# igorshmukler/kokoro-ruslan

Measured on AMD Instinct MI355X. Metric: mel-frames/sec (full train step), higher is better.
Workload: dtype bf16; 1 GPU; kokoro acoustic-model train step, 8x512 mel frames x 64 phonemes per GPU (BASELINE configs[1]), 49.4M params, fwd+loss+bwd+clip+AdamW+EMA every step; global_batch=8, frames=512, phonemes=64, parallelism=dp1, grad_allreduce=none (1 GPU), grad_accumulation=1, hipgraph=True

## Files before the change

### include/kokoro_hip.h

```cpp
#ifndef KOKORO_HIP_H
#define KOKORO_HIP_H
#include <stdint.h>
#ifdef __cplusplus
extern "C" {
#endif

#define KK_ABI_VERSION 2
#define KK_MATH_F32 0
#define KK_MATH_BF16 1
#define KK_EINVAL (-22)
#define KK_ENOTSUP (-95)
#define KK_SEG_ALIGN 1024

int kk_abi_version(void);
const char *kk_last_error(void);
const char *kk_last_kernel(void);

int kk_gemm(int ta, int tb, int64_t M, int64_t N, int64_t K, float alpha, const float *A, int64_t lda,
            const float *B, int64_t ldb, float beta, float *C, int64_t ldc, const float *bias,
            const float *residual, int64_t ldr, int64_t res_mod, int split_k, int math, int dtypes,
            void *stream);
typedef struct {
    const void *dy; int64_t lddy;
    const void *x;  int64_t ldx;
// ... 297 lines not shown
    double ema_decay;
    double max_weight_norm;
    int64_t ema_update_every;
    int64_t legacy_schedule;
    double legacy_cos, eta_min;
} KkOptCfg;
#define KK_OS_SKIPPED 0
#define KK_OS_EXPL_EMA 1
#define KK_OS_EXPL_EMA_STEPS 2
#define KK_OS_EXPL_STREAK 3
#define KK_OS_LAST_GRAD_NORM 4
#define KK_OS_LAST_CLIP_COEF 5
#define KK_OS_LAST_SKIP 6
#define KK_OS_LAST_BASE_LR 7
#define KK_OS_LAST_CLIP_NORM 8
#define KK_OS_EXPL_EMA_VALID 9
#define KK_OS_ATTEMPT 10
#define KK_OS_BAD_SEG 11
#define KK_OS_BAD_COUNT 12
#define KK_OS_BAD_ATTEMPT 13
#define KK_OS_MICRO_BAD 14
#define KK_OS_MICRO_BAD_TOTAL 15
#define KK_OS_SIZE 16
int64_t kk_seg_sumsq_ws_bytes(int64_t nblocks);
int64_t kk_seg_sumsq_rec_offset(void);
int kk_seg_sumsq_rec_capacity(void);
int kk_seg_sumsq(const float *buf, const int32_t *block_seg, int64_t nblocks, double *sumsq, int nseg, void *ws,
                 const int32_t *seg_skip, int extra_records, void *stream);
int kk_opt_prepare(const double *grad_sumsq, const float *seg_preclip, const float *seg_lr_mult,
                   const float *seg_wd, int nseg, const int64_t *max_dur, const KkOptCfg *cfg,
                   double *opt_state, float *seg_gscale, float *seg_decay, float *seg_stepsize,
                   float *step_consts ,
                   double *clear_a, double *clear_b , void *stream);
int kk_adamw_ema(float *p, const float *g, float *m, float *v, float *ema, const int32_t *block_seg,
                 int64_t nblocks, const float *seg_gscale, const float *seg_decay, const float *seg_stepsize,
                 const int32_t *seg_flags, const float *step_consts, float beta1, float beta2,
                 float ema_decay, int64_t *p_sumsq, int nseg, void *p_bf16, int zeroed, void *stream);
int kk_weight_norm_project(float *p, const int32_t *block_seg, int64_t nblocks, const int64_t *p_sumsq ,
                           const int32_t *seg_flags, const float *step_consts, double max_norm, void *p_bf16,
                           void *stream);
int kk_cast_f32_bf16(const float *src, void *dst, int64_t n, void *stream);

int kk_chain_begin(void *stream);
int kk_chain_launch(int kind, uint32_t *sync, uint64_t *trace, int flags, void *stream);
int kk_chain_abort(void *stream);

int kk_comm_load(const char *rccl_path );
int kk_comm_unique_id(void *id128);
int kk_comm_init(int rank, int world, const void *nccl_unique_id);
int kk_comm_world(void);
int kk_comm_destroy(void);
int kk_comm_reduce_bucket(void *ptr, int64_t count, int dtype, void *comm_stream);
int kk_comm_reduce_ranges(void *base, const int64_t *begin, const int64_t *end, int n, int dtype, void *comm_stream);
int kk_comm_loss_sync(double *acc, int n_acc, int64_t *max_dur, void *stream);
int kk_comm_reduce_scatter(const void *send, void *recv, int64_t recv_count, int dtype, void *comm_stream);
int kk_comm_all_gather(const void *send, void *recv, int64_t send_count, int dtype, void *comm_stream);
int kk_cast_bf16_f32(const void *x, float *y, int64_t n, float scale, void *stream);
int kk_cast_ranges(const void *src, void *dst, const int64_t *begin, const int64_t *end, int n, int to_bf16, float scale,
                   void *stream);

int kk_timestamp(uint64_t *slot, void *stream);
int kk_copy_many(const void *const *src, void *const *dst, const int64_t *bytes, int n, void *stream);
int kk_zero_many(void *const *dst, const int64_t *bytes, int n, void *stream);
int kk_axpby(float a, const float *x, float b, float *y, int64_t n, void *stream);
int kk_mfma_probe(float *out_f32 , float *out_bf16 , void *stream);

// ... 5 lines not shown
```

### include/kokoro_hip_tuning.h

```cpp
#ifndef KOKORO_HIP_TUNING_H
#define KOKORO_HIP_TUNING_H
#ifdef __cplusplus
extern "C" {
#endif
int kk_gemm_tune(int tm_threshold, int xcd_swizzle);
int kk_gemm_tune16(int enable, int thr128, int thr12864, int split_target);
int kk_gemm_tune_group(int split);
int kk_gemm_tune16x(int on, int force, int dbg);
#ifdef __cplusplus
}
#endif
#endif
```

### kokoro_ruslan_amd/csrc/kk_optim.hip

```cpp
#include "kk_common.h"
#include <math.h>

namespace {

constexpr int BLK = KK_SEG_ALIGN;
constexpr double KK_PSUMSQ_ONE = 1073741824.0;

typedef KkSegRec SegRec;
constexpr int SEG_REC_EXTRA = 4096;
constexpr int SEG_SUMSQ_WGS = 2048;

__global__ __launch_bounds__(256) void seg_sumsq_kernel(const float *__restrict__ buf, const int32_t *__restrict__ block_seg,
                                                        int64_t nblocks, int per_wg, double *__restrict__ sumsq, SegRec *__restrict__ rec,
                                                        const int32_t *__restrict__ skip) {
    __shared__ double red[4];
    __shared__ int32_t segs[256], skips[256];
    const int64_t beg = (int64_t)blockIdx.x * per_wg;
    const int64_t end = beg + per_wg < nblocks ? beg + per_wg : nblocks;
    SegRec lead = {0.0, -1, 0}, trail = {0.0, -1, 0};
    if (beg < end) {
        if (threadIdx.x < end - beg) {
            const int sg = block_seg[beg + threadIdx.x];
            segs[threadIdx.x] = sg;
            skips[threadIdx.x] = skip != nullptr ? skip[sg] : 0;
        }
        __syncthreads();
        int cur = segs[0];
        bool first = true;
        double acc = 0.0;
        bool cur_skip = skips[0] != 0;
        for (int64_t blk = beg; blk < end; ++blk) {
            const int seg = segs[blk - beg];
            if (seg != cur) {
                if (!cur_skip) {
                    const double tot = block_sum_256_d(acc, red);
                    if (first) { lead.v = tot; lead.seg = cur; first = false; }
                    else if (threadIdx.x == 0) sumsq[cur] = tot;
                }
                cur = seg;
                cur_skip = skips[blk - beg] != 0;
                acc = 0.0;
            }
            if (cur_skip) continue;
            const float4 v = ld4(buf + blk * BLK + threadIdx.x * 4);
            acc += (double)(v.x * v.x + v.y * v.y) + (double)(v.z * v.z + v.w * v.w);
        }
        if (!cur_skip) {
            const double tot = block_sum_256_d(acc, red);
            if (first) { lead.v = tot; lead.seg = cur; }
            else { trail.v = tot; trail.seg = cur; }
        }
    }
    if (threadIdx.x == 0) {
        rec[2 * blockIdx.x] = lead;
        rec[2 * blockIdx.x + 1] = trail;
    }
}

__device__ __forceinline__ void seg_merge16(const SegRec *in, int n, SegRec *out, double *sumsq, int t, bool last) {
    SegRec a = {0.0, -1, 0}, b = {0.0, -1, 0};
    int cur = -1;
    double acc = 0.0;
    bool have_first = false;
    for (int i = 16 * t; i < 16 * t + 16 && i < n; ++i) {
        const SegRec r = in[i];
        if (r.seg < 0) continue;
        if (r.seg != cur) {
            if (cur >= 0) {
                if (!have_first && !last) { a.v = acc; a.seg = cur; have_first = true; }
                else sumsq[cur] = acc;
            }
            cur = r.seg;
            acc = 0.0;
        }
        acc += r.v;
    }
    if (cur >= 0) {
        if (last) sumsq[cur] = acc;
        else if (!have_first) { a.v = acc; a.seg = cur; }
        else { b.v = acc; b.seg = cur; }
    }
    if (!last) { out[2 * t] = a; out[2 * t + 1] = b; }
}
__global__ __launch_bounds__(512) void seg_sumsq_finish_kernel(const SegRec *__restrict__ rec, int nrec, double *__restrict__ sumsq) {
    __shared__ SegRec l1[1024], l2[128], l3[16], l4[2];
    const int t = threadIdx.x;
    seg_merge16(rec, nrec, l1, sumsq, t, false);
    __syncthreads();
    if (t < 64) seg_merge16(l1, 1024, l2, sumsq, t, false);
    __syncthreads();
    if (t < 8) seg_merge16(l2, 128, l3, sumsq, t, false);
    __syncthreads();
    if (t == 0) seg_merge16(l3, 16, l4, sumsq, 0, true);
}

__device__ double onecycle_lr(const KkOptCfg &c, int64_t step_num) {
    const double total = (double)c.onecycle_steps;
    const double initial = c.max_lr / c.div_factor, min_lr = initial / c.final_div_factor;
    const double end1 = c.pct_start * total - 1.0, end2 = total - 1.0;
    const double PI = 3.14159265358979323846;
    if ((double)step_num <= end1) {
        if (end1 <= 0) return c.max_lr;
        return (initial - c.max_lr) / 2.0 * (cos(PI * ((double)step_num / end1)) + 1.0) + c.max_lr;
    }
    if (end2 <= end1) return min_lr;
    return (c.max_lr - min_lr) / 2.0 * (cos(PI * (((double)step_num - end1) / (end2 - end1))) + 1.0) + min_lr;
}

__device__ double base_lr_for(const KkOptCfg &c, int64_t k) {
    if (k == 0) return onecycle_lr(c, 0);
    const int64_t j = k - 1;
    if (c.use_warmup && j < c.warmup_steps)
        return c.warmup_start_lr + (c.warmup_target_lr - c.warmup_start_lr) * ((double)j / (double)c.warmup_steps);
    int64_t s = c.use_warmup ? j - c.warmup_steps + 1 : j + 1;
    if (s > c.onecycle_steps) s = c.onecycle_steps;
    return onecycle_lr(c, s);
}

__global__ __launch_bounds__(256) void opt_prepare_kernel(const double *__restrict__ grad_sumsq, const float *__restrict__ seg_preclip,
                                                          const float *__restrict__ seg_lr_mult, const float *__restrict__ seg_wd,
                                                          int nseg, const int64_t *__restrict__ max_dur, KkOptCfg c,
                                                          double *__restrict__ st, float *__restrict__ seg_gscale,
                                                          float *__restrict__ seg_decay, float *__restrict__ seg_stepsize,
                                                          float *__restrict__ step_consts, double *clear_a, double *clear_b) {
    __shared__ double red[4];
    __shared__ double sh[4];
    double part = 0.0, bad = 0.0;
    __shared__ int first_bad;
    if (threadIdx.x == 0) first_bad = 0x7fffffff;
    __syncthreads();
    for (int i = threadIdx.x; i < nseg; i += 256) {
        const double ss = grad_sumsq[i];
        const bool fin = isfinite(ss);
        if (!fin) atomicMin(&first_bad, i);
        double nr = sqrt(ss), sc = 1.0;
        const double pre = (double)seg_preclip[i];
        if (pre > 0.0 && fin && nr > pre) sc = pre / (nr + 1e-12);
        seg_gscale[i] = (float)sc;
        nr *= sc;
        part += nr * nr;
        if (!fin) bad += 1.0;
    }
    const double tot2 = block_sum_256_d(part, red);
    const double nbad = block_sum_256_d(bad, red);
    if (threadIdx.x == 0) {
        const double total = sqrt(tot2);
        double clip = c.max_grad_norm;
        const double md = max_dur ? (double)(*max_dur) : 0.0;
        const double risk = fmax((double)c.mel_length / 1400.0, md / 150.0);
        if (risk > 1.0) {
            clip = fmin(clip, fmax(0.3, 0.8 / pow(risk, 0.35)));
            clip = fmax(0.05, 0.5 / sqrt(risk));
        }
        const double attempt = st[KK_OS_ATTEMPT];
        const double done = attempt - st[KK_OS_SKIPPED];
        double floor_ = c.expl_abs_floor;
        if (c.expl_warmup_steps > 0 && done < (double)c.expl_warmup_steps)
            floor_ = c.expl_warmup_floor - (c.expl_warmup_floor - c.expl_abs_floor) * (done / (double)c.expl_warmup_steps);
        const bool ema_valid = st[KK_OS_EXPL_EMA_VALID] != 0.0;
        const bool ema_ready = st[KK_OS_EXPL_EMA_STEPS] >= (double)c.expl_min_ema_steps;
        const double ema_thr = ema_valid ? st[KK_OS_EXPL_EMA] * c.expl_multiplier : 0.0;
// ... 9 lines not shown
        const double coef = fmin(1.0, clip / (total + 1e-6));
        const double blr = c.legacy_schedule ? c.eta_min + (c.learning_rate - c.eta_min) * c.legacy_cos : base_lr_for(c, k);
        sh[0] = coef; sh[1] = blr; sh[2] = 1.0 - pow(c.beta1, (double)(k + 1)); sh[3] = skip ? 1.0 : 0.0;
        step_consts[0] = skip ? 1.f : (c.ema_update_every > 1 && k % c.ema_update_every != 0) ? 2.f : 0.f;
        step_consts[1] = (float)sqrt(1.0 - pow(c.beta2, (double)(k + 1)));
        step_consts[2] = (float)c.eps;
        step_consts[3] = (float)blr;
        st[KK_OS_ATTEMPT] = attempt + 1.0;
        if (skip) {
            st[KK_OS_SKIPPED] += 1.0;
            st[KK_OS_BAD_SEG] = (double)(first_bad + 1);
            st[KK_OS_BAD_COUNT] = nbad;
            st[KK_OS_BAD_ATTEMPT] = attempt;
        }
        st[KK_OS_LAST_GRAD_NORM] = total;
        st[KK_OS_LAST_CLIP_COEF] = coef;
        st[KK_OS_LAST_SKIP] = skip ? 1.0 : 0.0;
        st[KK_OS_LAST_BASE_LR] = blr;
        st[KK_OS_LAST_CLIP_NORM] = clip;
    }
    __syncthreads();
    const double coef = sh[0], blr = sh[1], bc1 = sh[2];
    for (int i = threadIdx.x; i < nseg; i += 256) {
        const double lr = c.legacy_schedule ? c.eta_min + (c.learning_rate * (double)seg_lr_mult[i] - c.eta_min) * c.legacy_cos
                                              : blr * (double)seg_lr_mult[i];
        seg_gscale[i] = (float)((double)seg_gscale[i] * coef);
        seg_decay[i] = (float)(1.0 - lr * (double)seg_wd[i]);
        seg_stepsize[i] = (float)(lr / bc1);
        if (clear_a) clear_a[i] = 0.0;
        if (clear_b) clear_b[i] = 0.0;
    }
}

__global__ __launch_bounds__(256) void adamw_ema_kernel(float *__restrict__ p, const float *__restrict__ g, float *__restrict__ m,
                                                        float *__restrict__ v, float *__restrict__ ema,
                                                        const int32_t *__restrict__ block_seg, const float *__restrict__ seg_gscale,
                                                        const float *__restrict__ seg_decay, const float *__restrict__ seg_stepsize,
                                                        const int32_t *__restrict__ seg_flags, const float *__restrict__ step_consts,
                                                        float beta1, float beta2, float ema_decay, unsigned long long *__restrict__ p_sumsq,
                                                        __bf16 *__restrict__ p16) {
    __shared__ float red[4];
    const float mode = step_consts[0];
    if (mode == 1.f) return;
    const int64_t blk = blockIdx.x;
    const int seg = block_seg[blk];
    const int flags = seg_flags[seg];
    const int64_t o = blk * BLK + threadIdx.x * 4;
    float4 pv = ld4(p + o);
    if (flags & 1) {
        const float gs = seg_gscale[seg], decay = seg_decay[seg], step = seg_stepsize[seg];
        const float bc2s = step_consts[1], eps = step_consts[2];
        const float4 gv = ld4(g + o);
        float4 mv = ld4(m + o), vv = ld4(v + o);
        float *pp = reinterpret_cast<float *>(&pv), *mp = reinterpret_cast<float *>(&mv), *vp = reinterpret_cast<float *>(&vv);
        const float *gp = reinterpret_cast<const float *>(&gv);
#pragma unroll
        for (int e = 0; e < 4; ++e) {
            const float gr = gp[e] * gs;
            float pe = pp[e] * decay;
            mp[e] = mp[e] + (1.f - beta1) * (gr - mp[e]);
            vp[e] = vp[e] * beta2 + (1.f - beta2) * gr * gr;
            const float denom = sqrtf(vp[e]) / bc2s + eps;
            pe = pe - step * (mp[e] / denom);
            pp[e] = pe;
        }
        st4(p + o, pv);
        st4(m + o, mv);
        st4(v + o, vv);
        if (p16) stv4<__bf16>(p16 + o, pv);
    }
    if ((flags & 2) && ema && mode == 0.f) {
        float4 ev = ld4(ema + o);
        const float w = 1.f - ema_decay;
        ev.x = ev.x * ema_decay + pv.x * w;
        ev.y = ev.y * ema_decay + pv.y * w;
        ev.z = ev.z * ema_decay + pv.z * w;
        ev.w = ev.w * ema_decay + pv.w * w;
        st4(ema + o, ev);
    }
    if ((flags & 4) && p_sumsq) {
        const float s = block_sum_256(pv.x * pv.x + pv.y * pv.y + pv.z * pv.z + pv.w * pv.w, red);
        if (threadIdx.x == 0) {
            const float sc = s < 4194304.f ? s : 4194304.f;
            atomicAdd(&p_sumsq[seg], (unsigned long long)((double)sc * KK_PSUMSQ_ONE + 0.5));
        }
    }
}

constexpr int WNP_BLOCKS = 8;
__global__ __launch_bounds__(256) void weight_norm_project_kernel(float *__restrict__ p, const int32_t *__restrict__ block_seg,
                                                                  const unsigned long long *__restrict__ p_sumsq, const int32_t *__restrict__ seg_flags,
                                                                  const float *__restrict__ step_consts, double max_norm,
                                                                  __bf16 *__restrict__ p16, int64_t nblocks) {
    __shared__ float scale[WNP_BLOCKS];
    if (step_consts[0] == 1.f) return;
    const int64_t b0 = (int64_t)blockIdx.x * WNP_BLOCKS;
    if (threadIdx.x < WNP_BLOCKS) {
        float sc = 0.f;
        const int64_t blk = b0 + threadIdx.x;
        if (blk < nblocks) {
            const int seg = block_seg[blk];
            if (seg_flags[seg] & 4) {
                const double nr = sqrt((double)p_sumsq[seg] * (1.0 / KK_PSUMSQ_ONE));
                if (nr > max_norm) sc = (float)(max_norm / nr);
            }
        }
        scale[threadIdx.x] = sc;
    }
    __syncthreads();
#pragma unroll
    for (int j = 0; j < WNP_BLOCKS; ++j) {
        const float sc = scale[j];
        if (sc == 0.f) continue;
        const int64_t o = (b0 + j) * BLK + threadIdx.x * 4;
        float4 pv = ld4(p + o);
        pv.x *= sc; pv.y *= sc; pv.z *= sc; pv.w *= sc;
        st4(p + o, pv);
        if (p16) stv4<__bf16>(p16 + o, pv);
    }
}

__global__ __launch_bounds__(256) void cast_bf16_kernel(const float *__restrict__ src, __bf16 *__restrict__ dst, int64_t n4) {
    for (int64_t i = (int64_t)blockIdx.x * 256 + threadIdx.x; i < n4; i += (int64_t)gridDim.x * 256) stv4<__bf16>(dst + 4 * i, ld4(src + 4 * i));
}

}

extern "C" int64_t kk_seg_sumsq_ws_bytes(int64_t nblocks) {
    (void)nblocks;
    return (int64_t)sizeof(SegRec) * (2 * SEG_SUMSQ_WGS + SEG_REC_EXTRA);
}
extern "C" int64_t kk_seg_sumsq_rec_offset(void) { return (int64_t)sizeof(SegRec) * 2 * SEG_SUMSQ_WGS; }
extern "C" int kk_seg_sumsq_rec_capacity(void) { return SEG_REC_EXTRA; }

extern "C" int kk_seg_sumsq(const float *buf, const int32_t *block_seg, int64_t nblocks, double *sumsq, int nseg, void *ws,
                            const int32_t *seg_skip, int extra_records, void *stream) {
    KK_REQUIRE(buf && block_seg && sumsq && ws && nblocks > 0 && nseg > 0, "kk_seg_sumsq: bad args (the record workspace is required)");
    KK_REQUIRE(extra_records >= 0 && extra_records <= SEG_REC_EXTRA && (extra_records == 0 || seg_skip != nullptr),
               "kk_seg_sumsq: %d tile records (0..%d, with a skip table)", extra_records, SEG_REC_EXTRA);
    hipStream_t s = (hipStream_t)stream;
    const int wgs = SEG_SUMSQ_WGS;
    const int per = kk_cdiv(nblocks, wgs);
    KK_REQUIRE(per <= 256, "kk_seg_sumsq: arenas beyond %d blocks are not supported", 256 * SEG_SUMSQ_WGS);
    SegRec *rec = static_cast<SegRec *>(ws);
    hipLaunchKernelGGL(seg_sumsq_kernel, dim3(wgs), dim3(256), 0, s, buf, block_seg, nblocks, per, sumsq, rec, seg_skip);
    hipLaunchKernelGGL(seg_sumsq_finish_kernel, dim3(1), dim3(512), 0, s, rec, 2 * SEG_SUMSQ_WGS + extra_records, sumsq);
    KK_LAUNCH_CHECK("kk_seg_sumsq");
    return 0;
}

extern "C" int kk_opt_prepare(const double *grad_sumsq, const float *seg_preclip, const float *seg_lr_mult,
                              const float *seg_wd, int nseg, const int64_t *max_dur, const KkOptCfg *cfg,
                              double *opt_state, float *seg_gscale, float *seg_decay, float *seg_stepsize,
                              float *step_consts, double *clear_a, double *clear_b, void *stream) {
    KK_REQUIRE(grad_sumsq && seg_preclip && seg_lr_mult && seg_wd && cfg && opt_state && nseg > 0, "kk_opt_prepare: bad args");
    hipLaunchKernelGGL(opt_prepare_kernel, dim3(1), dim3(256), 0, (hipStream_t)stream, grad_sumsq, seg_preclip, seg_lr_mult,
                       seg_wd, nseg, max_dur, *cfg, opt_state, seg_gscale, seg_decay, seg_stepsize, step_consts, clear_a, clear_b);
    KK_LAUNCH_CHECK("kk_opt_prepare");
    return 0;
}

extern "C" int kk_adamw_ema(float *p, const float *g, float *m, float *v, float *ema, const int32_t *block_seg,
                            int64_t nblocks, const float *seg_gscale, const float *seg_decay,
                            const float *seg_stepsize, const int32_t *seg_flags, const float *step_consts,
                            float beta1, float beta2, float ema_decay, int64_t *p_sumsq, int nseg, void *p_bf16,
                            int zeroed, void *stream) {
    KK_REQUIRE(p && g && m && v && block_seg && nblocks > 0 && nblocks < (1ll << 31), "kk_adamw_ema: bad args");
    hipStream_t s = (hipStream_t)stream;
    if (p_sumsq && !zeroed) {
        const int e = kk_zero_async(p_sumsq, sizeof(int64_t) * nseg, s);
        if (e != 0) return e;
    }
    hipLaunchKernelGGL(adamw_ema_kernel, dim3((unsigned)nblocks), dim3(256), 0, s, p, g, m, v, ema, block_seg, seg_gscale,
                       seg_decay, seg_stepsize, seg_flags, step_consts, beta1, beta2, ema_decay, reinterpret_cast<unsigned long long *>(p_sumsq),
                       reinterpret_cast<__bf16 *>(p_bf16));
    KK_LAUNCH_CHECK("kk_adamw_ema");
    return 0;
}

extern "C" int kk_weight_norm_project(float *p, const int32_t *block_seg, int64_t nblocks, const int64_t *p_sumsq,
                                      const int32_t *seg_flags, const float *step_consts, double max_norm,
                                      void *p_bf16, void *stream) {
    KK_REQUIRE(p && block_seg && p_sumsq && seg_flags && nblocks > 0, "kk_weight_norm_project: bad args");
    if (!(max_norm > 0.0)) return 0;
    hipLaunchKernelGGL(weight_norm_project_kernel, dim3((unsigned)kk_cdiv(nblocks, WNP_BLOCKS)), dim3(256), 0, (hipStream_t)stream, p,
                       block_seg, reinterpret_cast<const unsigned long long *>(p_sumsq), seg_flags, step_consts, max_norm,
                       reinterpret_cast<__bf16 *>(p_bf16), nblocks);
    KK_LAUNCH_CHECK("kk_weight_norm_project");
    return 0;
}

extern "C" int kk_cast_f32_bf16(const float *src, void *dst, int64_t n, void *stream) {
    KK_REQUIRE(src && dst && n > 0 && n % 4 == 0, "kk_cast_f32_bf16: n must be a positive multiple of 4");
    int blocks = kk_cdiv(n / 4, 256);
    if (blocks > 4096) blocks = 4096;
    hipLaunchKernelGGL(cast_bf16_kernel, dim3(blocks), dim3(256), 0, (hipStream_t)stream, src, reinterpret_cast<__bf16 *>(dst), n / 4);
    KK_LAUNCH_CHECK("kk_cast_f32_bf16");
    return 0;
}
```

### kokoro_ruslan_amd/engine.py

```python
from __future__ import annotations

import contextlib
import math
import os
import threading
from collections import OrderedDict
from typing import Dict, Optional, Sequence, Tuple

import torch

from . import lib as kk
from . import spec
from .spec import VA, ModelDims, StepHyper

CHUNK = 512
_ITEMSIZE = {torch.float32: 4, torch.bfloat16: 2, torch.float64: 8, torch.int64: 8, torch.int32: 4, torch.uint8: 1}


def _b16(t) -> int:
    return 1 if t is not None and t.dtype == torch.bfloat16 else 0


class Arena:

# ... 108 lines not shown
        self.train_dropout = False
        self.overlap = True
        self._side = torch.cuda.Stream(device=self.device)
        self._tmp_ns = ""
        self._kv = torch.cuda.Stream(device=self.device)
        self.dec_head_aside = True
        self.tail_aside = -1
        self.embed_bwd_sorted = True
        self.wgrad0_aside = -1
        self.lr_epoch = 0
        self.fuse_glu_fwd = True
        self.group_wgrads = True
        self.fuse_headnorm = True
        self.fuse_headnorm_bwd = True
        self.attn_bwd_pair = True
        self.attn_two_pass = True
        self.attn_keep_bits = True
        self.attn_keep_gen = True
        self.attn_keep_gen_rate = 1100.0
        self.grad_norm_from_wgrads = True
        self._ss_step = None
        self._ss_ready = None
        self._ss_masks: Dict[frozenset, torch.Tensor] = {}
        self._external_sync = False
        self._seg_of_ptr = {self.arena.G[n].data_ptr(): i for i, n in enumerate(self.arena.names)}
        self.attn_warm = 5
        self._keep_ready = set()
        self.attn_pair_min_seq = 64
        self.attn_proj_bf16 = True
        self.fuse_linear_tail = True
        self._acc_clean = True
        self._acc_depth = 0
        self._self_cleaning_acc = True
        self.fuse_enc_prologue = True
        self.rowdot_partials = True
        self.fuse_memory_fwd = True
        self.zero_skip_overwritten = True
        self._ow_sets: Dict[Tuple, frozenset] = {}
        self._ow_seen: Optional[set] = None
        self._ow_expect: Optional[frozenset] = None
        self._wgrad_queue = {}
        self._defer_wgrads = None
        self._grads_fresh = False
        self._first_micro = False
        self.enc_fused = True
        self.enc_fused_max_batch = 8
        self.zero_late = True
        self.enc_placement = 0
        self._enc_sync = torch.zeros(512, dtype=torch.int32, device=self.device)
        self.enc_trace, self.enc_trace_wg = None, 0
        self.spec_augment_active = True
        self.trace = os.environ.get("KK_TRACE", "0") == "1"
        self._marks: Dict[str, int] = {}
        self._mark_buf = torch.zeros(512, dtype=torch.int64, device=self.device) if self.trace else None
        self.rng = torch.full((1,), int(seed) & 0x7FFFFFFF, dtype=torch.int32, device=self.device)
        for n, b in spec.make_buffers(self.dims).items():
            self.arena.P[n].copy_(b)
        if init:
            self.load_params(spec.init_params(self.dims, seed))
        elif self.arena.ema is not None:
            self.arena.ema.copy_(self.arena.p)
        self.sync_shadow()

    @property
    def self_cleaning_acc(self) -> bool:
        return self._self_cleaning_acc

    @self_cleaning_acc.setter
    def self_cleaning_acc(self, on) -> None:
        if bool(on) != self._self_cleaning_acc:
            self._acc_clean = False
        self._self_cleaning_acc = bool(on)

    @contextlib.contextmanager
    def _acc_guard(self):
        if self._acc_depth == 0:
            if not self._acc_clean:
                if torch.cuda.is_current_stream_capturing():
                    raise RuntimeError("the step's accumulators are not in their zero state inside a graph capture")
                self.loss_acc.zero_()
                self.grad_sumsq.zero_()
                self.p_sumsq.zero_()
            self._acc_clean = False
        self._acc_depth += 1
        try:
            yield
        except BaseException:
            self._acc_depth -= 1
            raise
        self._acc_depth -= 1
        if self._acc_depth == 0:
            self._acc_clean = True

    def load_params(self, params: Dict[str, torch.Tensor], reset_ema: bool = True) -> None:
        for n in self.arena.param_names:
            self.arena.P[n].copy_(params[n].to(self.device, torch.float32).view(self.arena.shapes[n]))
        if reset_ema and self.arena.ema is not None:
            self.arena.ema.copy_(self.arena.p)
        self.sync_shadow()

    @contextlib.contextmanager
    def fp32_math(self):
        saved = (self.math, self.enc_dt, self.dec_dt, self.use_shadow)
        self.math, self.enc_dt, self.dec_dt, self.use_shadow = kk.KK_MATH_F32, torch.float32, torch.float32, False
        try:
            yield self
        finally:
            self.math, self.enc_dt, self.dec_dt, self.use_shadow = saved

    @contextlib.contextmanager
    def ema_weights(self):
        a = self.arena
        if a.ema is None:
            yield self
            return
# ... 1364 lines not shown
            self.zero_grad()
            return
        self._ow_expect = rec

        def build():
            base, spans, pos = a.g.data_ptr(), [], 0
            for ptr, n in sorted(rec):
                b = (ptr - base) // 4
                if b < pos or b % 4 or n % 4:
                    raise RuntimeError("overlapping or misaligned weight-gradient tensors in the overwrite record")
                if b > pos:
                    spans.append(a.g[pos:b])
                pos = b + n
            if pos < a.total:
                spans.append(a.g[pos:a.total])
            return [kk.zero_table(spans[i:i + 160]) for i in range(0, len(spans), 160)]
        for dst, nbytes, n in self._table(("zero", a.g.data_ptr(), rec), build):
            kk.call("kk_zero_many", dst, nbytes, n)

    def optimizer_step(self, mel_length: int, tile_norms=None) -> None:
        a, hp = self.arena, self.hp
        cfg = self._opt_cfg(mel_length)
        self._mark("optimizer start")
        skip, extra = None, 0
        if tile_norms is not None and tile_norms[1] > 0:
            skip = self._ss_masks.get(tile_norms[0])
            if skip is None and not torch.cuda.is_current_stream_capturing():
                m = torch.zeros(a.nseg, dtype=torch.int32)
                m[sorted(tile_norms[0])] = 1
                skip = self._ss_masks[tile_norms[0]] = m.to(self.device)
            extra = tile_norms[1] if skip is not None else 0
        with self._acc_guard():
            sc = 1 if self.self_cleaning_acc else 0
            kk.call("kk_seg_sumsq", a.g, a.block_seg, a.nblocks, self.grad_sumsq, a.nseg, self.sumsq_ws, skip, extra)
            kk.call("kk_opt_prepare", self.grad_sumsq, a.seg_preclip, a.seg_lr_mult, a.seg_wd, a.nseg, self.max_dur, cfg,
                    self.opt_state, self.seg_gscale, self.seg_decay, self.seg_stepsize, self.step_consts,
                    None, self.p_sumsq if sc else None)
            kk.call("kk_adamw_ema", a.p, a.g, a.m, a.v, a.ema, a.block_seg, a.nblocks, self.seg_gscale, self.seg_decay,
                    self.seg_stepsize, a.seg_flags, self.step_consts, hp.adam_betas[0], hp.adam_betas[1], hp.ema_decay,
                    self.p_sumsq, a.nseg, a.p16, sc)
            kk.call("kk_weight_norm_project", a.p, a.block_seg, a.nblocks, self.p_sumsq, a.seg_flags, self.step_consts,
                    float(hp.dec_ffn_max_weight_norm), a.p16)
        self._mark("optimizer done")

    def train_step(self, batch: Dict[str, torch.Tensor], accumulation_divisor: Optional[int] = None,
                   boundary: Optional[bool] = None, grad_sync=None, expanded_len: Optional[int] = None) -> torch.Tensor:
        G = max(1, int(self.hp.gradient_accumulation_steps))
        div = accumulation_divisor if accumulation_divisor is not None else G
        if self.micro_in_cycle == 0:
            self.zero_grad()
        is_boundary = bool(boundary) if boundary is not None else self.micro_in_cycle + 1 >= G
        self._exchange_now = is_boundary
        self._first_micro = self.micro_in_cycle == 0
        self._external_sync = grad_sync is not None
        try:
            out = self.forward_backward(batch, loss_scale=self.dp_loss_scale / div, adaptive=True, expanded_len=expanded_len)
        finally:
            self._first_micro = False
            self._external_sync = False
        self._exchange_now = True
        self.micro_in_cycle += 1
        if is_boundary:
            if grad_sync is not None:
                grad_sync(self.arena.g)
            self.optimizer_step(canonical_mel_length(self.global_mel_length, batch["mel_specs"].shape[1]),
                                self._ss_ready if grad_sync is None else None)
            self._ss_ready = None
            self.micro_in_cycle = 0
        return out["losses"]

# ... 65 lines not shown
            if v.data_ptr() == d.data_ptr():
                continue
            if v.shape == d.shape and v.dtype == d.dtype and v.device == d.device and v.is_contiguous() and d.is_contiguous():
                moved.append((d, v))
            else:
                d.copy_(v, non_blocking=True)
        if moved:
            kk.copy_many(moved)
        fkey = (div, first, self.train_dropout, self.spec_augment_active, self.math, self.dp_comm is not None and is_boundary,
                mel_length if self.loss_sync is not None else 0, self.loss_sync is not None, self.self_cleaning_acc, (self.attn_keep_gen, self.attn_keep_gen_rate),
                self.grad_norm_from_wgrads and grad_sync is None)
        with self._acc_guard():
            fbe = ent["fb"].get(fkey)
            if fbe is None:
                with self.capture_lock:
                    self._external_sync = grad_sync is not None
                    try:
                        g_ = self._capture_fb(static, scale, first, expanded_len)
                    finally:
                        self._external_sync = False
                    fbe = ent["fb"][fkey] = (g_, self._ss_ready)
            self._exchange_now = True
            fbe[0].replay()
            self._ss_ready = fbe[1]
        self.micro_in_cycle += 1
        if grad_sync is not None and is_boundary:
            grad_sync(self.arena.g)
        if is_boundary:
            epoch = 0 if self.hp.use_onecycle_lr else self.lr_epoch
            tn = self._ss_ready if grad_sync is None else None
            self._ss_ready = None
            if tn is not None and tn[0] not in self._ss_masks:
                tn = None
            okey = (mel_length, epoch, self.self_cleaning_acc, tn)
            for k in [k for k in ent["opt"] if k[1] != epoch]:
                torch.cuda.synchronize(self.device)
                del ent["opt"][k]
            with self._acc_guard():
                opt = ent["opt"].get(okey)
                if opt is None:
                    with self.capture_lock:
                        torch.cuda.synchronize()
                        opt = ent["opt"][okey] = torch.cuda.CUDAGraph()
                        with torch.cuda.graph(opt, capture_error_mode="thread_local"):
                            self.optimizer_step(mel_length, tn)
                opt.replay()
            self.micro_in_cycle = 0
        return self.losses

    def encoder_stack_error(self) -> int:
        return int(self._enc_sync[0].item())

    def check_encoder_stack(self) -> None:
        import torch.distributed as dist
        multi = dist.is_available() and dist.is_initialized() and dist.get_world_size() > 1
        if not self.enc_fused and not multi:
            return
        code = self.encoder_stack_error() if self.enc_fused else 0
        if multi:
            word = torch.tensor([code], dtype=torch.int64, device=self.device if dist.get_backend() == "nccl" else "cpu")
            dist.all_reduce(word, op=dist.ReduceOp.MAX)
            code = int(word.item())
        if code:
            self._enc_sync.zero_()
            if self.enc_fused:
                self.enc_fused = False
                self._graphs.clear()
# ... 8 lines not shown
```

### kokoro_ruslan_amd/lib.py

```python
from __future__ import annotations

import ctypes as C
import os
from typing import Any, Dict, List

import torch

HERE = os.path.dirname(os.path.abspath(__file__))
LIB_PATH = os.path.join(HERE, "libkokoro_hip.so")

KK_MATH_F32, KK_MATH_BF16 = 0, 1
KK_SEG_ALIGN = 1024
OS = dict(SKIPPED=0, EXPL_EMA=1, EXPL_EMA_STEPS=2, EXPL_STREAK=3, LAST_GRAD_NORM=4, LAST_CLIP_COEF=5,
          LAST_SKIP=6, LAST_BASE_LR=7, LAST_CLIP_NORM=8, EXPL_EMA_VALID=9, ATTEMPT=10, BAD_SEG=11, BAD_COUNT=12,
          BAD_ATTEMPT=13, MICRO_BAD=14, MICRO_BAD_TOTAL=15, SIZE=16)


class KkLossCfg(C.Structure):
    _fields_ = [("w_dur", C.c_float), ("w_stop", C.c_float), ("w_pitch", C.c_float), ("w_energy", C.c_float),
                ("delta_dur", C.c_float), ("delta_pitch", C.c_float), ("delta_energy", C.c_float),
                ("pos_weight", C.c_float), ("loss_scale", C.c_float), ("adaptive", C.c_int)]


class KkOptCfg(C.Structure):
# ... 177 lines not shown
    "kk_encoder_stack_fwd": [C.POINTER(KkEncStack), _P],
    "kk_dropout_bwd": [_P, _P, _L, _I, _I, _P, _U, _F, _U, _F, _U, _F, _I, _P],
    "kk_specaug": [_P, _I, _I, _I, _P, _U, _I, _I, _I, _I, _I, _P],
    "kk_ids_eq_zero": [_P, _P, _L, _P],
    "kk_shift_right": [_P, _P, _I, _I, _I, _P],
    "kk_decode_prologue": [_P, _P, _P, _P, _P, _P, _P, _P, _P, _P, _I, _I, _I, _I, _P],
    "kk_decode_cache_append": [_P, _P, _P, _P, _P, _I, _I, _I, _P],
    "kk_decode_epilogue": [_P, _P, _P, _P, _P, _I, _I, _I, _P],
    "kk_im2col3_rows_fwd": [_P, _P, _P, _I, _I, _I, _I, _I, _P],
    "kk_groupnorm_relu_rows_fwd": [_P, _P, _P, _P, _P, _P, _P, _I, _I, _I, _I, _P, _U, _F, _P],
    "kk_varpred_row_mask": [_P, _P, _P, _I, _I, _I, _P],
    "kk_decode_epilogue_rows": [_P, _P, _P, _P, _P, _P, _P, _P, _P, _P, _P, _I, _I, _I, _F, _F, _P],
    "kk_voc_conv1d": [_P, _L, _I, _P, _I, _I, _P, _P, _I, _I, _I, _F, _P, _I, _P, _P, _I, _I, _P],
    "kk_voc_convt1d": [_P, _L, _I, _P, _I, _I, _P, _P, _I, _I, _I, _F, _P, _I, _I, _P],
    "kk_voc_convt_taps": [_I, _I, _P],
    "kk_voc_post": [_P, _L, _I, _P, _P, _P, _I, _F, _P, _I, _P],
    "kk_gl_tile_frames": [],
    "kk_gl_init": [_P, _L, _P, _P, _P, _P, _P, _P],
    "kk_gl_iter": [_P, _P, _P, _P, _P, _I, _P, _P, _F, _P],
    "kk_gl_istft": [_P, _P, _I, _P, _P, _P, _P],
    "kk_feat_mel_tile_frames": [],
    "kk_feat_peak": [_P, _P, _I, _L, _P, _P],
    "kk_feat_mel": [_P, _P, _P, _P, _P, _I, _P, _P, _P, _P, _P, _P, _P, _P],
    "kk_feat_pitch": [_P, _P, _P, _P, _P, _I, _P, _P, _P, _P, _P],
    "kk_feat_finish": [_P, _P, _I, _P, _P, _P, _P, _P, _P, _P, _P, _I, _P],
    "kk_losses_fwd": [_P] * 12 + [_I, _I, _I, _I, C.POINTER(KkLossCfg), _P, _P, _P, _P, _P, _I, _P],
    "kk_losses_finalize": [_P, C.POINTER(KkLossCfg), _P, _I, _P, _P, _P, _I, _P],
    "kk_losses_bwd": [_P] * 12 + [_I, _I, _I, _I, C.POINTER(KkLossCfg), _P, _P, _P, _P, _P, _P, _P],
    "kk_chain_begin": [_P],
    "kk_chain_launch": [_I, _P, _P, _I, _P],
    "kk_chain_abort": [_P],
    "kk_seg_sumsq": [_P, _P, _L, _P, _I, _P, _P, _I, _P],
    "kk_opt_prepare": [_P, _P, _P, _P, _I, _P, C.POINTER(KkOptCfg), _P, _P, _P, _P, _P, _P, _P, _P],
    "kk_adamw_ema": [_P, _P, _P, _P, _P, _P, _L, _P, _P, _P, _P, _P, _F, _F, _F, _P, _I, _P, _I, _P],
    "kk_weight_norm_project": [_P, _P, _L, _P, _P, _P, _D, _P, _P],
    "kk_cast_f32_bf16": [_P, _P, _L, _P],
    "kk_comm_load": [C.c_char_p],
    "kk_comm_unique_id": [_P],
    "kk_comm_init": [_I, _I, _P],
    "kk_comm_world": [],
    "kk_comm_destroy": [],
    "kk_comm_reduce_bucket": [_P, _L, _I, _P],
    "kk_comm_reduce_ranges": [_P, _P, _P, _I, _I, _P],
    "kk_comm_loss_sync": [_P, _I, _P, _P],
    "kk_comm_reduce_scatter": [_P, _P, _L, _I, _P],
    "kk_comm_all_gather": [_P, _P, _L, _I, _P],
    "kk_cast_bf16_f32": [_P, _P, _L, _F, _P],
    "kk_cast_ranges": [_P, _P, _P, _P, _I, _I, _F, _P],
    "kk_copy_many": [_P, _P, _P, _I, _P],
    "kk_axpby": [_F, _P, _F, _P, _L, _P],
    "kk_timestamp": [_P, _P],
    "kk_mfma_probe": [_P, _P, _P],
}

_lib = None
_prof = None


def profile_start() -> None:
    global _prof
    _prof = []


def profile_stop():
    global _prof
    rec, _prof = _prof or [], None
# ... 105 lines not shown
```

Measured before the change: 1.167 million mel-frames/s.

## Fuse grad segment norm and optimizer prepare into one last-block kernel

Merges the per-segment gradient sum-of-squares walk, the record merge and opt_prepare into one kernel: the last workgroup, found through an atomic ticket, does the merge and the prepare. This removes one or two launches and their serialization gaps. It also prefetches 8 blocks ahead in the segment walk and rewrites the AdamW kernel as a grid-strided loop with next-block prefetch, with optional non-temporal stores. By default the AdamW grid still equals nblocks and temporal stores are used. The ticket needs zeroing in the workspace tail, and correctness relies on threadfence ordering.

Result: slower. 1.144 million mel-frames/s (-2.0%).

```diff
diff --git a/include/kokoro_hip.h b/include/kokoro_hip.h
--- a/include/kokoro_hip.h
+++ b/include/kokoro_hip.h
@@ -353,6 +353,10 @@
                    double *opt_state, float *seg_gscale, float *seg_decay, float *seg_stepsize,
                    float *step_consts ,
                    double *clear_a, double *clear_b , void *stream);
+int kk_opt_norm_prepare(const float *buf, const int32_t *block_seg, int64_t nblocks, double *grad_sumsq, int nseg, void *ws,
+                        const int32_t *seg_skip, int extra_records, const float *seg_preclip, const float *seg_lr_mult,
+                        const float *seg_wd, const int64_t *max_dur, const KkOptCfg *cfg, double *opt_state, float *seg_gscale,
+                        float *seg_decay, float *seg_stepsize, float *step_consts, double *clear_a, double *clear_b, void *stream);
 int kk_adamw_ema(float *p, const float *g, float *m, float *v, float *ema, const int32_t *block_seg,
                  int64_t nblocks, const float *seg_gscale, const float *seg_decay, const float *seg_stepsize,
                  const int32_t *seg_flags, const float *step_consts, float beta1, float beta2,
diff --git a/include/kokoro_hip_tuning.h b/include/kokoro_hip_tuning.h
--- a/include/kokoro_hip_tuning.h
+++ b/include/kokoro_hip_tuning.h
@@ -1,11 +1,17 @@
 #ifndef KOKORO_HIP_TUNING_H
 #define KOKORO_HIP_TUNING_H
+#include <stdint.h>
 #ifdef __cplusplus
 extern "C" {
 #endif
 int kk_gemm_tune(int tm_threshold, int xcd_swizzle);
 int kk_gemm_tune16(int enable, int thr128, int thr12864, int split_target);
 int kk_gemm_tune_group(int split);
+int kk_adamw_tune(int grid_wgs, int nt);
+int kk_adamw_ema_ref(float *p, const float *g, float *m, float *v, float *ema, const int32_t *block_seg, int64_t nblocks,
+                     const float *seg_gscale, const float *seg_decay, const float *seg_stepsize, const int32_t *seg_flags,
+                     const float *step_consts, float beta1, float beta2, float ema_decay, int64_t *p_sumsq, int nseg, void *p_bf16,
+                     int zeroed, void *stream);
 int kk_gemm_tune16x(int on, int force, int dbg);
 #ifdef __cplusplus
 }
diff --git a/kokoro_ruslan_amd/csrc/kk_optim.hip b/kokoro_ruslan_amd/csrc/kk_optim.hip
--- a/kokoro_ruslan_amd/csrc/kk_optim.hip
+++ b/kokoro_ruslan_amd/csrc/kk_optim.hip
@@ -9,12 +9,12 @@
 typedef KkSegRec SegRec;
 constexpr int SEG_REC_EXTRA = 4096;
 constexpr int SEG_SUMSQ_WGS = 2048;
-
-__global__ __launch_bounds__(256) void seg_sumsq_kernel(const float *__restrict__ buf, const int32_t *__restrict__ block_seg,
-                                                        int64_t nblocks, int per_wg, double *__restrict__ sumsq, SegRec *__restrict__ rec,
-                                                        const int32_t *__restrict__ skip) {
-    __shared__ double red[4];
-    __shared__ int32_t segs[256], skips[256];
+constexpr int SEG_TICKET_BYTES = 64;
+
+constexpr int SEG_WALK_AHEAD = 8;
+__device__ __forceinline__ void seg_walk(const float *__restrict__ buf, const int32_t *__restrict__ block_seg, int64_t nblocks, int per_wg,
+                                         double *sumsq, SegRec *rec, const int32_t *__restrict__ skip, double *red, int32_t *segs,
+                                         int32_t *skips) {
     const int64_t beg = (int64_t)blockIdx.x * per_wg;
     const int64_t end = beg + per_wg < nblocks ? beg + per_wg : nblocks;
     SegRec lead = {0.0, -1, 0}, trail = {0.0, -1, 0};
@@ -29,21 +29,32 @@
         bool first = true;
         double acc = 0.0;
         bool cur_skip = skips[0] != 0;
-        for (int64_t blk = beg; blk < end; ++blk) {
-            const int seg = segs[blk - beg];
-            if (seg != cur) {
-                if (!cur_skip) {
-                    const double tot = block_sum_256_d(acc, red);
-                    if (first) { lead.v = tot; lead.seg = cur; first = false; }
-                    else if (threadIdx.x == 0) sumsq[cur] = tot;
+        for (int64_t b0 = beg; b0 < end; b0 += SEG_WALK_AHEAD) {
+            float4 pre[SEG_WALK_AHEAD];
+#pragma unroll
+            for (int j = 0; j < SEG_WALK_AHEAD; ++j) {
+                const int64_t blk = b0 + j;
+                pre[j] = blk < end && skips[blk - beg] == 0 ? ld4(buf + blk * BLK + threadIdx.x * 4) : make_float4(0.f, 0.f, 0.f, 0.f);
+            }
+#pragma unroll
+            for (int j = 0; j < SEG_WALK_AHEAD; ++j) {
+                const int64_t blk = b0 + j;
+                if (blk >= end) break;
+                const int seg = segs[blk - beg];
+                if (seg != cur) {
+                    if (!cur_skip) {
+                        const double tot = block_sum_256_d(acc, red);
+                        if (first) { lead.v = tot; lead.seg = cur; first = false; }
+                        else if (threadIdx.x == 0) sumsq[cur] = tot;
+                    }
+                    cur = seg;
+                    cur_skip = skips[blk - beg] != 0;
+                    acc = 0.0;
                 }
-                cur = seg;
-                cur_skip = skips[blk - beg] != 0;
-                acc = 0.0;
+                if (cur_skip) continue;
+                const float4 v = pre[j];
+                acc += (double)(v.x * v.x + v.y * v.y) + (double)(v.z * v.z + v.w * v.w);
             }
-            if (cur_skip) continue;
-            const float4 v = ld4(buf + blk * BLK + threadIdx.x * 4);
-            acc += (double)(v.x * v.x + v.y * v.y) + (double)(v.z * v.z + v.w * v.w);
         }
         if (!cur_skip) {
             const double tot = block_sum_256_d(acc, red);
@@ -55,6 +66,14 @@
         rec[2 * blockIdx.x] = lead;
         rec[2 * blockIdx.x + 1] = trail;
     }
+}
+
+__global__ __launch_bounds__(256) void seg_sumsq_kernel(const float *__restrict__ buf, const int32_t *__restrict__ block_seg,
+                                                        int64_t nblocks, int per_wg, double *__restrict__ sumsq, SegRec *__restrict__ rec,
+                                                        const int32_t *__restrict__ skip) {
+    __shared__ double red[4];
+    __shared__ int32_t segs[256], skips[256];
+    seg_walk(buf, block_seg, nblocks, per_wg, sumsq, rec, skip, red, segs, skips);
 }
 
 __device__ __forceinline__ void seg_merge16(const SegRec *in, int n, SegRec *out, double *sumsq, int t, bool last) {
@@ -117,16 +136,15 @@
     return onecycle_lr(c, s);
 }
 
-__global__ __launch_bounds__(256) void opt_prepare_kernel(const double *__restrict__ grad_sumsq, const float *__restrict__ seg_preclip,
-                                                          const float *__restrict__ seg_lr_mult, const float *__restrict__ seg_wd,
-                                                          int nseg, const int64_t *__restrict__ max_dur, KkOptCfg c,
-                                                          double *__restrict__ st, float *__restrict__ seg_gscale,
-                                                          float *__restrict__ seg_decay, float *__restrict__ seg_stepsize,
-                                                          float *__restrict__ step_consts, double *clear_a, double *clear_b) {
-    __shared__ double red[4];
-    __shared__ double sh[4];
+__device__ __forceinline__ void opt_prepare_body(const double *grad_sumsq, const float *__restrict__ seg_preclip,
+                                                 const float *__restrict__ seg_lr_mult, const float *__restrict__ seg_wd, int nseg,
+                                                 const int64_t *__restrict__ max_dur, const KkOptCfg &c, double *__restrict__ st,
+                                                 float *__restrict__ seg_gscale, float *__restrict__ seg_decay,
+                                                 float *__restrict__ seg_stepsize, float *__restrict__ step_consts, double *clear_a,
+                                                 double *clear_b, double *red, double *sh ,
+                                                 int *first_bad_p) {
+    int &first_bad = *first_bad_p;
     double part = 0.0, bad = 0.0;
-    __shared__ int first_bad;
     if (threadIdx.x == 0) first_bad = 0x7fffffff;
     __syncthreads();
     for (int i = threadIdx.x; i < nseg; i += 256) {
@@ -202,7 +220,63 @@
     }
 }
 
-__global__ __launch_bounds__(256) void adamw_ema_kernel(float *__restrict__ p, const float *__restrict__ g, float *__restrict__ m,
+__global__ __launch_bounds__(256) void opt_prepare_kernel(const double *__restrict__ grad_sumsq, const float *__restrict__ seg_preclip,
+                                                          const float *__restrict__ seg_lr_mult, const float *__restrict__ seg_wd,
+                                                          int nseg, const int64_t *__restrict__ max_dur, KkOptCfg c,
+                                                          double *__restrict__ st, float *__restrict__ seg_gscale,
+                                                          float *__restrict__ seg_decay, float *__restrict__ seg_stepsize,
+                                                          float *__restrict__ step_consts, double *clear_a, double *clear_b) {
+    __shared__ double red[4];
+    __shared__ double sh[4];
+    __shared__ int first_bad;
+    opt_prepare_body(grad_sumsq, seg_preclip, seg_lr_mult, seg_wd, nseg, max_dur, c, st, seg_gscale, seg_decay, seg_stepsize, step_consts,
+                     clear_a, clear_b, red, sh, &first_bad);
+}
+
+struct NormPrepareShared {
+    SegRec l1[1024], l2[128], l3[16], l4[2];
+    double red[4], sh[4];
+    int32_t segs[256], skips[256];
+    int first_bad;
+    unsigned last;
+};
+__global__ __launch_bounds__(256) void seg_norm_prepare_kernel(const float *__restrict__ buf, const int32_t *__restrict__ block_seg,
+                                                               int64_t nblocks, int per_wg, double *sumsq, SegRec *rec,
+                                                               const int32_t *__restrict__ skip, int nrec, unsigned *ticket,
+                                                               const float *__restrict__ seg_preclip, const float *__restrict__ seg_lr_mult,
+                                                               const float *__restrict__ seg_wd, int nseg,
+                                                               const int64_t *__restrict__ max_dur, KkOptCfg c, double *__restrict__ st,
+                                                               float *__restrict__ seg_gscale, float *__restrict__ seg_decay,
+                                                               float *__restrict__ seg_stepsize, float *__restrict__ step_consts,
+                                                               double *clear_a, double *clear_b) {
+    __shared__ NormPrepareShared sm;
+    seg_walk(buf, block_seg, nblocks, per_wg, sumsq, rec, skip, sm.red, sm.segs, sm.skips);
+    if (threadIdx.x == 0) {
+        __threadfence();
+        sm.last = atomicAdd(ticket, 1u) == gridDim.x - 1 ? 1u : 0u;
+    }
+    __syncthreads();
+    if (sm.last == 0u) return;
+    __threadfence();
+    const int t = threadIdx.x;
+    seg_merge16(rec, nrec, sm.l1, sumsq, t, false);
+    seg_merge16(rec, nrec, sm.l1, sumsq, t + 256, false);
+    __syncthreads();
+    if (t < 64) seg_merge16(sm.l1, 1024, sm.l2, sumsq, t, false);
+    __syncthreads();
+    if (t < 8) seg_merge16(sm.l2, 128, sm.l3, sumsq, t, false);
+    __syncthreads();
+    if (t == 0) {
+        seg_merge16(sm.l3, 16, sm.l4, sumsq, 0, true);
+        *ticket = 0u;
+    }
+    __syncthreads();
+    opt_prepare_body(sumsq, seg_preclip, seg_lr_mult, seg_wd, nseg, max_dur, c, st, seg_gscale, seg_decay, seg_stepsize, step_consts,
+                     clear_a, clear_b, sm.red, sm.sh, &sm.first_bad);
+}
+
+#ifdef KK_TUNING_HOOKS
+__global__ __launch_bounds__(256) void adamw_ema_ref_kernel(float *__restrict__ p, const float *__restrict__ g, float *__restrict__ m,
                                                         float *__restrict__ v, float *__restrict__ ema,
                                                         const int32_t *__restrict__ block_seg, const float *__restrict__ seg_gscale,
                                                         const float *__restrict__ seg_decay, const float *__restrict__ seg_stepsize,
@@ -256,6 +330,82 @@
         }
     }
 }
+#endif
+
+typedef float kk_f32x4 __attribute__((ext_vector_type(4)));
+template <bool NT> __device__ __forceinline__ void st4_state(float *p, float4 v) {
+    if (NT) __builtin_nontemporal_store(__builtin_bit_cast(kk_f32x4, v), reinterpret_cast<kk_f32x4 *>(p));
+    else st4(p, v);
+}
+constexpr int ADAMW_GRID_DEFAULT = 0, ADAMW_NT_DEFAULT = 0;
+template <bool NT>
+__global__ __launch_bounds__(256) void adamw_ema_kernel(float *__restrict__ p, const float *__restrict__ g, float *__restrict__ m,
+                                                        float *__restrict__ v, float *__restrict__ ema,
+                                                        const int32_t *__restrict__ block_seg, const float *__restrict__ seg_gscale,
+                                                        const float *__restrict__ seg_decay, const float *__restrict__ seg_stepsize,
+                                                        const int32_t *__restrict__ seg_flags, const float *__restrict__ step_consts,
+                                                        float beta1, float beta2, float ema_decay, unsigned long long *__restrict__ p_sumsq,
+                                                        __bf16 *__restrict__ p16, int64_t nblocks) {
+    __shared__ float red[4];
+    int64_t blk = blockIdx.x;
+    int64_t o = blk * BLK + threadIdx.x * 4;
+    float4 pv = ld4(p + o), gv = ld4(g + o), mv = ld4(m + o), vv = ld4(v + o);
+    int seg = block_seg[blk];
+    const float mode = step_consts[0];
+    const float bc2s = step_consts[1], eps = step_consts[2];
+    for (;;) {
+        const int64_t nb = blk + gridDim.x;
+        const bool more = nb < nblocks && mode != 1.f;
+        const int64_t on = nb * BLK + threadIdx.x * 4;
+        float4 pn = make_float4(0.f, 0.f, 0.f, 0.f), gn = pn, mn = pn, vn = pn;
+        int segn = 0;
+        if (more) {
+            pn = ld4(p + on); gn = ld4(g + on); mn = ld4(m + on); vn = ld4(v + on);
+            segn = block_seg[nb];
+        }
+        const int flags = mode == 1.f ? 0 : seg_flags[seg];
+        const bool do_ema = (flags & 2) && ema && mode == 0.f;
+        float4 ev = make_float4(0.f, 0.f, 0.f, 0.f);
+        if (do_ema) ev = ld4(ema + o);
+        if (flags & 1) {
+            const float gs = seg_gscale[seg], decay = seg_decay[seg], step = seg_stepsize[seg];
+            float *pp = reinterpret_cast<float *>(&pv), *mp = reinterpret_cast<float *>(&mv), *vp = reinterpret_cast<float *>(&vv);
+            const float *gp = reinterpret_cast<const float *>(&gv);
+#pragma unroll
+            for (int e = 0; e < 4; ++e) {
+                const float gr = gp[e] * gs;
+                float pe = pp[e] * decay;
+                mp[e] = mp[e] + (1.f - beta1) * (gr - mp[e]);
+                vp[e] = vp[e] * beta2 + (1.f - beta2) * gr * gr;
+                const float denom = sqrtf(vp[e]) / bc2s + eps;
+                pe = pe - step * (mp[e] / denom);
+                pp[e] = pe;
+            }
+            st4(p + o, pv);
+            st4_state<NT>(m + o, mv);
+            st4_state<NT>(v + o, vv);
+            if (p16) stv4<__bf16>(p16 + o, pv);
+        }
+        if (do_ema) {
+            const float w = 1.f - ema_decay;
+            ev.x = ev.x * ema_decay + pv.x * w;
+            ev.y = ev.y * ema_decay + pv.y * w;
+            ev.z = ev.z * ema_decay + pv.z * w;
+            ev.w = ev.w * ema_decay + pv.w * w;
+            st4_state<NT>(ema + o, ev);
+        }
+        if ((flags & 4) && p_sumsq) {
+            const float s = block_sum_256(pv.x * pv.x + pv.y * pv.y + pv.z * pv.z + pv.w * pv.w, red);
+            if (threadIdx.x == 0) {
+                const float sc = s < 4194304.f ? s : 4194304.f;
+                atomicAdd(&p_sumsq[seg], (unsigned long long)((double)sc * KK_PSUMSQ_ONE + 0.5));
+            }
+        }
+        if (!more) break;
+        blk = nb; o = on; seg = segn;
+        pv = pn; gv = gn; mv = mn; vv = vn;
+    }
+}
 
 constexpr int WNP_BLOCKS = 8;
 __global__ __launch_bounds__(256) void weight_norm_project_kernel(float *__restrict__ p, const int32_t *__restrict__ block_seg,
@@ -296,9 +446,18 @@
 
 }
 
+static int g_adamw_grid = ADAMW_GRID_DEFAULT, g_adamw_nt = ADAMW_NT_DEFAULT;
+#ifdef KK_TUNING_HOOKS
+extern "C" int kk_adamw_tune(int grid_wgs, int nt) {
+    g_adamw_grid = grid_wgs < 0 ? ADAMW_GRID_DEFAULT : grid_wgs;
+    g_adamw_nt = nt < 0 ? ADAMW_NT_DEFAULT : (nt != 0);
+    return 0;
+}
+#endif
+
 extern "C" int64_t kk_seg_sumsq_ws_bytes(int64_t nblocks) {
     (void)nblocks;
-    return (int64_t)sizeof(SegRec) * (2 * SEG_SUMSQ_WGS + SEG_REC_EXTRA);
+    return (int64_t)sizeof(SegRec) * (2 * SEG_SUMSQ_WGS + SEG_REC_EXTRA) + SEG_TICKET_BYTES;
 }
 extern "C" int64_t kk_seg_sumsq_rec_offset(void) { return (int64_t)sizeof(SegRec) * 2 * SEG_SUMSQ_WGS; }
 extern "C" int kk_seg_sumsq_rec_capacity(void) { return SEG_REC_EXTRA; }
@@ -330,6 +489,29 @@
     return 0;
 }
 
+extern "C" int kk_opt_norm_prepare(const float *buf, const int32_t *block_seg, int64_t nblocks, double *grad_sumsq, int nseg, void *ws,
+                                   const int32_t *seg_skip, int extra_records, const float *seg_preclip, const float *seg_lr_mult,
+                                   const float *seg_wd, const int64_t *max_dur, const KkOptCfg *cfg, double *opt_state,
+                                   float *seg_gscale, float *seg_decay, float *seg_stepsize, float *step_consts, double *clear_a,
+                                   double *clear_b, void *stream) {
+    KK_REQUIRE(buf && block_seg && grad_sumsq && ws && nblocks > 0 && nseg > 0, "kk_opt_norm_prepare: bad args (the record workspace is required)");
+    KK_REQUIRE(extra_records >= 0 && extra_records <= SEG_REC_EXTRA && (extra_records == 0 || seg_skip != nullptr),
+               "kk_opt_norm_prepare: %d tile records (0..%d, with a skip table)", extra_records, SEG_REC_EXTRA);
+    KK_REQUIRE(seg_preclip && seg_lr_mult && seg_wd && cfg && opt_state && seg_gscale && seg_decay && seg_stepsize && step_consts,
+               "kk_opt_norm_prepare: bad args");
+    KK_REQUIRE(clear_a != grad_sumsq && clear_b != grad_sumsq, "kk_opt_norm_prepare: grad_sumsq is this launch's own output");
+    const int wgs = SEG_SUMSQ_WGS;
+    const int per = kk_cdiv(nblocks, wgs);
+    KK_REQUIRE(per <= 256, "kk_opt_norm_prepare: arenas beyond %d blocks are not supported", 256 * SEG_SUMSQ_WGS);
+    SegRec *rec = static_cast<SegRec *>(ws);
+    unsigned *ticket = reinterpret_cast<unsigned *>(rec + 2 * SEG_SUMSQ_WGS + SEG_REC_EXTRA);
+    hipLaunchKernelGGL(seg_norm_prepare_kernel, dim3(wgs), dim3(256), 0, (hipStream_t)stream, buf, block_seg, nblocks, per, grad_sumsq, rec,
+                       seg_skip, 2 * SEG_SUMSQ_WGS + extra_records, ticket, seg_preclip, seg_lr_mult, seg_wd, nseg, max_dur, *cfg, opt_state,
+                       seg_gscale, seg_decay, seg_stepsize, step_consts, clear_a, clear_b);
+    KK_LAUNCH_CHECK("kk_opt_norm_prepare");
+    return 0;
+}
+
 extern "C" int kk_adamw_ema(float *p, const float *g, float *m, float *v, float *ema, const int32_t *block_seg,
                             int64_t nblocks, const float *seg_gscale, const float *seg_decay,
                             const float *seg_stepsize, const int32_t *seg_flags, const float *step_consts,
@@ -341,12 +523,36 @@
         const int e = kk_zero_async(p_sumsq, sizeof(int64_t) * nseg, s);
         if (e != 0) return e;
     }
-    hipLaunchKernelGGL(adamw_ema_kernel, dim3((unsigned)nblocks), dim3(256), 0, s, p, g, m, v, ema, block_seg, seg_gscale,
+    const int grid_wgs = g_adamw_grid, nt = g_adamw_nt;
+    const unsigned grid = grid_wgs > 0 && grid_wgs < nblocks ? (unsigned)grid_wgs : (unsigned)nblocks;
+#define KK_ADAMW(NT)                                                                                                              \
+    hipLaunchKernelGGL(adamw_ema_kernel<NT>, dim3(grid), dim3(256), 0, s, p, g, m, v, ema, block_seg, seg_gscale, seg_decay,     \
+                       seg_stepsize, seg_flags, step_consts, beta1, beta2, ema_decay, reinterpret_cast<unsigned long long *>(p_sumsq), \
+                       reinterpret_cast<__bf16 *>(p_bf16), nblocks)
+    if (nt) KK_ADAMW(true); else KK_ADAMW(false);
+#undef KK_ADAMW
+    KK_LAUNCH_CHECK("kk_adamw_ema");
+    return 0;
+}
+
+#ifdef KK_TUNING_HOOKS
+extern "C" int kk_adamw_ema_ref(float *p, const float *g, float *m, float *v, float *ema, const int32_t *block_seg, int64_t nblocks,
+                                const float *seg_gscale, const float *seg_decay, const float *seg_stepsize, const int32_t *seg_flags,
+                                const float *step_consts, float beta1, float beta2, float ema_decay, int64_t *p_sumsq, int nseg,
+                                void *p_bf16, int zeroed, void *stream) {
+    KK_REQUIRE(p && g && m && v && block_seg && nblocks > 0 && nblocks < (1ll << 31), "kk_adamw_ema_ref: bad args");
+    hipStream_t s = (hipStream_t)stream;
+    if (p_sumsq && !zeroed) {
+        const int e = kk_zero_async(p_sumsq, sizeof(int64_t) * nseg, s);
+        if (e != 0) return e;
+    }
+    hipLaunchKernelGGL(adamw_ema_ref_kernel, dim3((unsigned)nblocks), dim3(256), 0, s, p, g, m, v, ema, block_seg, seg_gscale,
                        seg_decay, seg_stepsize, seg_flags, step_consts, beta1, beta2, ema_decay, reinterpret_cast<unsigned long long *>(p_sumsq),
                        reinterpret_cast<__bf16 *>(p_bf16));
-    KK_LAUNCH_CHECK("kk_adamw_ema");
-    return 0;
-}
+    KK_LAUNCH_CHECK("kk_adamw_ema_ref");
+    return 0;
+}
+#endif
 
 extern "C" int kk_weight_norm_project(float *p, const int32_t *block_seg, int64_t nblocks, const int64_t *p_sumsq,
                                       const int32_t *seg_flags, const float *step_consts, double max_norm,
diff --git a/kokoro_ruslan_amd/engine.py b/kokoro_ruslan_amd/engine.py
--- a/kokoro_ruslan_amd/engine.py
+++ b/kokoro_ruslan_amd/engine.py
@@ -164,6 +164,7 @@
         self._acc_clean = True
         self._acc_depth = 0
         self._self_cleaning_acc = True
+        self.fuse_norm_prepare = True
         self.fuse_enc_prologue = True
         self.rowdot_partials = True
         self.fuse_memory_fwd = True
@@ -213,6 +214,7 @@
                 self.loss_acc.zero_()
                 self.grad_sumsq.zero_()
                 self.p_sumsq.zero_()
+                self.sumsq_ws[-64:].zero_()
             self._acc_clean = False
         self._acc_depth += 1
         try:
@@ -1643,10 +1645,15 @@
             extra = tile_norms[1] if skip is not None else 0
         with self._acc_guard():
             sc = 1 if self.self_cleaning_acc else 0
-            kk.call("kk_seg_sumsq", a.g, a.block_seg, a.nblocks, self.grad_sumsq, a.nseg, self.sumsq_ws, skip, extra)
-            kk.call("kk_opt_prepare", self.grad_sumsq, a.seg_preclip, a.seg_lr_mult, a.seg_wd, a.nseg, self.max_dur, cfg,
-                    self.opt_state, self.seg_gscale, self.seg_decay, self.seg_stepsize, self.step_consts,
-                    None, self.p_sumsq if sc else None)
+            if self.fuse_norm_prepare:
+                kk.call("kk_opt_norm_prepare", a.g, a.block_seg, a.nblocks, self.grad_sumsq, a.nseg, self.sumsq_ws, skip, extra,
+                        a.seg_preclip, a.seg_lr_mult, a.seg_wd, self.max_dur, cfg, self.opt_state, self.seg_gscale, self.seg_decay,
+                        self.seg_stepsize, self.step_consts, None, self.p_sumsq if sc else None)
+            else:
+                kk.call("kk_seg_sumsq", a.g, a.block_seg, a.nblocks, self.grad_sumsq, a.nseg, self.sumsq_ws, skip, extra)
+                kk.call("kk_opt_prepare", self.grad_sumsq, a.seg_preclip, a.seg_lr_mult, a.seg_wd, a.nseg, self.max_dur, cfg,
+                        self.opt_state, self.seg_gscale, self.seg_decay, self.seg_stepsize, self.step_consts,
+                        None, self.p_sumsq if sc else None)
             kk.call("kk_adamw_ema", a.p, a.g, a.m, a.v, a.ema, a.block_seg, a.nblocks, self.seg_gscale, self.seg_decay,
                     self.seg_stepsize, a.seg_flags, self.step_consts, hp.adam_betas[0], hp.adam_betas[1], hp.ema_decay,
                     self.p_sumsq, a.nseg, a.p16, sc)
@@ -1778,7 +1785,7 @@
             self._ss_ready = None
             if tn is not None and tn[0] not in self._ss_masks:
                 tn = None
-            okey = (mel_length, epoch, self.self_cleaning_acc, tn)
+            okey = (mel_length, epoch, self.self_cleaning_acc, tn, self.fuse_norm_prepare)
             for k in [k for k in ent["opt"] if k[1] != epoch]:
                 torch.cuda.synchronize(self.device)
                 del ent["opt"][k]
diff --git a/kokoro_ruslan_amd/lib.py b/kokoro_ruslan_amd/lib.py
--- a/kokoro_ruslan_amd/lib.py
+++ b/kokoro_ruslan_amd/lib.py
@@ -233,6 +233,7 @@
     "kk_chain_abort": [_P],
     "kk_seg_sumsq": [_P, _P, _L, _P, _I, _P, _P, _I, _P],
     "kk_opt_prepare": [_P, _P, _P, _P, _I, _P, C.POINTER(KkOptCfg), _P, _P, _P, _P, _P, _P, _P, _P],
+    "kk_opt_norm_prepare": [_P, _P, _L, _P, _I, _P, _P, _I, _P, _P, _P, _P, C.POINTER(KkOptCfg), _P, _P, _P, _P, _P, _P, _P, _P],
     "kk_adamw_ema": [_P, _P, _P, _P, _P, _P, _L, _P, _P, _P, _P, _P, _F, _F, _F, _P, _I, _P, _I, _P],
     "kk_weight_norm_project": [_P, _P, _L, _P, _P, _P, _D, _P, _P],
     "kk_cast_f32_bf16": [_P, _P, _L, _P],
```
